# aswanthabam/JPEG_Decoder

Hardware: AMD Instinct MI355X
Metric: Mpixels/s decoded (IDCT+colour) (higher is better)
Workload: dtype f32; 1 GPU; stream of 4096x4096 baseline 4:4:4 images, 32 images per step (one launch) per GPU, coefficient blocks resident in HBM; sampling=4:4:4, parallelism=images sharded x1, no collective, launched_by=bench.py

## Files before the change

jpeg_decoder_amd/csrc/jb_huff.hip:

```cpp
#include <hip/hip_runtime.h>
#include <stdint.h>

#include "jb_huff_core.h"
#include "jb_kernels.h"

namespace {

constexpr uint32_t L = kJbhLanes;
constexpr int kMaxPasses = (int)L + 4;

__constant__ uint8_t kZz2Dev[64] = {0,   2,   16,  32,  18,  4,   6,   20,  34,  48, 64,  50,  36,  22,  8,   10,
                                    24,  38,  52,  66,  80,  96,  82,  68,  54,  40, 26,  12,  14,  28,  42,  56,
                                    70,  84,  98,  112, 114, 100, 86,  72,  58,  44, 30,  46,  60,  74,  88,  102,
                                    116, 118, 104, 90,  76,  62,  78,  92,  106, 120, 122, 108, 94,  110, 124, 126};

template <uint32_t kMaxChunk>
struct Lay {
  static constexpr uint32_t kRows = jbh_rows(kMaxChunk);
  static constexpr uint32_t kNcp = kMaxChunk * 8u / kJbCheckpointBits;
  static_assert(kNcp <= kJbCheckpoints, "records per chunk");
  static constexpr uint32_t off_stream = 0;
  static constexpr uint32_t off_cp = off_stream + kRows * L * 4u;
  static constexpr uint32_t off_xbit = off_cp + kNcp * L * 4u;
  static constexpr uint32_t off_xmeta = off_xbit + L * 4u;
  static constexpr uint32_t off_misc = off_xmeta + L * 4u;
  static constexpr uint32_t off_tab = off_misc + 256u;
  static uint32_t bytes(uint32_t n_tabs) { return off_tab + n_tabs * kJbT1Entries * 2u + kJbT2Tables * kJbT2Entries * 2u; }
};

struct ChunkGeo {
  uint32_t start, end;
  uint32_t seg;
  bool first, last;
};
__device__ __forceinline__ ChunkGeo chunk_geo(const JbHuffLaunch &p, const JbHuffImage &img, uint32_t gidx) {
  const JbChunkDesc cd = p.chunks[gidx];
  ChunkGeo x;
  x.seg = cd.seg & 0x7fffffffu;
  x.first = (cd.seg >> 31) != 0;
  uint32_t seg_end = p.starts[img.int_off + x.seg + 1];
  if (seg_end > img.scan_len) seg_end = img.scan_len;
  x.start = cd.start < seg_end ? cd.start : seg_end;
  x.end = x.start + img.chunk_bytes < seg_end ? x.start + img.chunk_bytes : seg_end;
  x.last = x.end == seg_end;
  return x;
}

template <uint32_t kRows>
__device__ __forceinline__ void load_stream(uint32_t *stream, const uint8_t *img_scan, uint32_t start, uint32_t tid) {
  const uint8_t *src = img_scan + (int32_t)jbh_base_byte(start);
#pragma unroll
  for (uint32_t q = 0; q < (kRows + 3u) / 4u; q++) {
    const uint4 v = *(const uint4 *)(src + 16u * q);
    const uint32_t d[4] = {v.x, v.y, v.z, v.w};
#pragma unroll
    for (uint32_t i = 0; i < 4; i++)
      if (4u * q + i < kRows) stream[(4u * q + i) * L + tid] = __builtin_bswap32(d[i]);
  }
}

__device__ __forceinline__ void load_tables(uint16_t *tab, const JbHuffLaunch &p, const JbHuffImage &img, uint32_t tid) {
  const JbHuffTables *set = p.tables + img.table_set;
  const uint4 *s1 = (const uint4 *)set->t1;
  uint4 *d = (uint4 *)tab;
  const uint32_t n1 = img.n_tabs * kJbT1Entries * 2u / 16u;
  for (uint32_t i = tid; i < n1; i += L) d[i] = s1[i];
  const uint4 *s2 = (const uint4 *)set->t2;
  constexpr uint32_t n2 = kJbT2Tables * kJbT2Entries * 2u / 16u;
  for (uint32_t i = tid; i < n2; i += L) d[n1 + i] = s2[i];
}

struct Seg {
  uint32_t f, n, d0, d1, d2;
};
__device__ __forceinline__ Seg seg_combine(const Seg &a, const Seg &b) {
  Seg r;
  r.f = a.f | b.f;
  r.n = b.f ? b.n : a.n + b.n;
  r.d0 = b.f ? b.d0 : a.d0 + b.d0;
  r.d1 = b.f ? b.d1 : a.d1 + b.d1;
  r.d2 = b.f ? b.d2 : a.d2 + b.d2;
  return r;
}
__device__ __forceinline__ Seg seg_shfl_up(const Seg &x, int off) {
  Seg r;
  r.f = __shfl_up(x.f, off);
  r.n = __shfl_up(x.n, off);
  r.d0 = __shfl_up(x.d0, off);
  r.d1 = __shfl_up(x.d1, off);
  r.d2 = __shfl_up(x.d2, off);
  return r;
}
__device__ __forceinline__ Seg seg_scan_wg(Seg x, uint32_t *scratch, uint32_t tid, Seg *total) {
  const uint32_t lane = tid & 63u, wave = tid >> 6;
#pragma unroll
  for (int off = 1; off < 64; off <<= 1) {
    const Seg t = seg_shfl_up(x, off);
    if (lane >= (uint32_t)off) x = seg_combine(t, x);
  }
  __syncthreads();
  if (lane == 63u) {
    uint32_t *s = scratch + wave * 5u;
    s[0] = x.f, s[1] = x.n, s[2] = x.d0, s[3] = x.d1, s[4] = x.d2;
  }
  __syncthreads();
  Seg run{0, 0, 0, 0, 0};
  Seg all{0, 0, 0, 0, 0};
#pragma unroll
  for (uint32_t w = 0; w < L / 64u; w++) {
    const uint32_t *s = scratch + w * 5u;
    const Seg t{s[0], s[1], s[2], s[3], s[4]};
    if (w < wave) run = seg_combine(run, t);
    all = seg_combine(all, t);
  }
  *total = all;
  return seg_combine(run, x);
}

__device__ __forceinline__ Seg fold_left_workgroups(const JbHuffLaunch &p, uint32_t w_first, uint32_t w_me, uint32_t *red, uint32_t tid) {
  if (tid < 8) red[tid] = 0;
  __syncthreads();
  uint32_t last_f = 0;
  for (uint32_t w = w_first + tid; w < w_me; w += L)
    if (p.wgsum[w].has_first) last_f = w - w_first + 1u;
  if (last_f) atomicMax(&red[0], last_f);
  __syncthreads();
  const uint32_t from = red[0];
  uint32_t a_n = 0, a0 = 0, a1 = 0, a2 = 0;
  for (uint32_t w = w_first + tid; w < w_me; w += L) {
    if (w - w_first + 1u >= from) {
      const JbWgSum s = p.wgsum[w];
      a_n += s.blocks, a0 += s.dc[0], a1 += s.dc[1], a2 += s.dc[2];
    }
  }
  if (a_n) atomicAdd(&red[1], a_n);
  if (a0) atomicAdd(&red[2], a0);
  if (a1) atomicAdd(&red[3], a1);
  if (a2) atomicAdd(&red[4], a2);
  __syncthreads();
  return Seg{from ? 1u : 0u, red[1], red[2], red[3], red[4]};
}
__device__ __forceinline__ Seg scan_left(const Seg &mine, const Seg &carry, uint32_t *scratch, uint32_t tid, Seg *total) {
  const Seg incl = seg_scan_wg(mine, scratch, tid, total);
  Seg left = seg_shfl_up(incl, 1);
  if ((tid & 63u) == 0) {
    left = Seg{0, 0, 0, 0, 0};
    for (uint32_t w = 0; w < (tid >> 6); w++) {
      const uint32_t *s = scratch + w * 5u;
      left = seg_combine(left, Seg{s[0], s[1], s[2], s[3], s[4]});
    }
  }
  return seg_combine(carry, left);
}

}

constexpr uint32_t kMet = 0x80000000u;

template <uint32_t kMaxChunk>
__global__ __launch_bounds__(kJbHuffLanes) void jb_huff_sync_kernel(const JbHuffLaunch p, const int launch) {
  using Ly = Lay<kMaxChunk>;
  extern __shared__ __attribute__((aligned(16))) uint8_t lds[];
  uint32_t *const stream = (uint32_t *)(lds + Ly::off_stream);
  uint32_t *const cpst = (uint32_t *)(lds + Ly::off_cp);
  uint32_t *const xbit = (uint32_t *)(lds + Ly::off_xbit);
  uint32_t *const xmeta = (uint32_t *)(lds + Ly::off_xmeta);
  uint32_t *const misc = (uint32_t *)(lds + Ly::off_misc);
  uint16_t *const tab = (uint16_t *)(lds + Ly::off_tab);
  const uint32_t tid = threadIdx.x;
  const JbHuffWg wg = p.sync_wgs[blockIdx.x];
  const JbHuffImage img = p.images[wg.image];
  const uint32_t ci = wg.first_chunk + tid - kJbWarmChunks;
  const bool owned = tid >= kJbWarmChunks && ci < img.n_chunks;
  const bool active = ci < img.n_chunks && (owned || launch == 0);
  const uint32_t gidx = img.state_off + (ci < img.n_chunks ? ci : img.n_chunks - 1u);
  const ChunkGeo g = chunk_geo(p, img, gidx);
  const uint32_t u0 = jbh_u_of_bit(g.start, g.start * 8u), u_end = u0 + (g.end - g.start) * 8u;
  const size_t n_all = p.n_chunks_total;

  JbChunkState entry{g.start * 8u, 0u}, exitst{0u, 0u};
  bool changed = active;
  if (launch > 0) {
    bool c0 = false;
    JbChunkState ne{0u, 0u};
    if (tid == kJbWarmChunks && owned && !g.first) {
      ne = p.exit[gidx - 1u];
      const JbChunkState en = p.entry[gidx];
      c0 = ne.bitpos != en.bitpos || ((ne.meta ^ en.meta) & 0xffffu) != 0;
    }
    if (!__syncthreads_or(c0)) return;
    entry = p.entry[gidx];
    exitst = p.exit[gidx];
    changed = c0;
    if (c0) entry = JbChunkState{ne.bitpos, ne.meta & 0xffffu};
  }
  load_tables(tab, p, img, tid);
  if (active) load_stream<Ly::kRows>(stream, p.scan + img.scan_off, g.start, tid);
#pragma unroll
  for (uint32_t i = 0; i < Ly::kNcp; i++) cpst[i * L + tid] = launch > 0 ? p.cps[i * n_all + gidx] : 0xffffffffu;
  __syncthreads();

  JbhCtx cx;
  cx.scol = stream + tid;
  cx.tab = tab;
  cx.zz2 = nullptr;
  cx.lut_ac = img.lut_ac, cx.lut_dc = img.lut_dc, cx.lut_comp = img.lut_comp;
  cx.nb4 = img.nb * 4u;
  cx.blk_bytes = img.blk_bytes;
  cx.t2_first = img.n_tabs * kJbT1Entries;
  uint32_t *const cpl = cpst + tid;

  for (int pass = 0; pass < kMaxPasses; pass++) {
    if (__builtin_amdgcn_ballot_w64(changed) != 0) {
      JbhLane st;
      {
        const uint32_t bit = entry.bitpos < g.start * 8u ? g.start * 8u : entry.bitpos;
        const uint32_t u = jbh_u_of_bit(g.start, bit);
        st.u = (changed && u < u_end) ? u : u_end;
        st.k = entry.meta & 0xffu;
        st.blk4 = ((entry.meta >> 8) & 0xffu) * 4u;
        if (st.k > 63u) st.k = 0;
        if (st.blk4 >= cx.nb4) st.blk4 = 0;
        st.nblk = 0;
      }
      uint32_t none = 0;
      while (st.u < u_end) {
        const uint32_t up = st.u;
        (void)jbh_step<false>(cx, st, none, none, none, nullptr, 0u);
        if (((st.u ^ up) >> 8) != 0) {
          uint32_t *rec = cpl + ((st.u >> 8) - 1u) * L;
          const uint32_t s = jbh_pack_state(st), old = *rec;
          const bool met = (st.u < u_end) & (((old ^ s) & 0xfffffu) == 0);
          *rec = met ? old : s;
          st.u = met ? (kMet | ((st.u >> 8) - 1u)) : st.u;
        }
      }
      JBH_TRACE_PASS_END(pass);
      if (changed) {
        if (st.u >= kMet) {
          const uint32_t met_i = st.u & 0xffu;
          const uint32_t dn = st.nblk - (cpl[met_i * L] >> 20);
          for (uint32_t i = met_i; i < Ly::kNcp; i++) cpl[i * L] += dn << 20;
          exitst.meta = (exitst.meta & 0xffffu) | ((((exitst.meta >> 16) + dn) & 0xffffu) << 16);
        } else {
          exitst.bitpos = jbh_bit_of_u(g.start, st.u);
          exitst.meta = st.k | (st.blk4 << 6) | ((st.nblk & 0xffffu) << 16);
        }
      }
    }
    xbit[tid] = exitst.bitpos;
    xmeta[tid] = exitst.meta & 0xffffu;
    __syncthreads();
    changed = false;
    if (active && !g.first && tid > (launch == 0 ? 0u : kJbWarmChunks)) {
      const uint32_t nbit = xbit[tid - 1u], nmeta = xmeta[tid - 1u];
      if (nbit != entry.bitpos || nmeta != (entry.meta & 0xffffu)) {
        entry = JbChunkState{nbit, nmeta};
        changed = true;
      }
    }
    if (!__syncthreads_or(changed)) break;
  }
  if (owned) {
    p.entry[gidx] = entry;
    p.exit[gidx] = exitst;
#pragma unroll
    for (uint32_t i = 0; i < Ly::kNcp; i++) p.cps[i * n_all + gidx] = cpl[i * L];
  }
  Seg mine{0, 0, 0, 0, 0};
  if (owned) {
    mine.f = g.first ? 1u : 0u;
    mine.n = (exitst.meta >> 16) + (g.first ? g.seg * img.ri * img.nb : 0u);
  }
  Seg total;
  (void)seg_scan_wg(mine, misc + 16, tid, &total);
  if (tid == 0) {
    JbWgSum *o = p.wgsum + img.wg0 + wg.first_chunk / kJbOwnChunks;
    o->has_first = total.f;
    o->blocks = total.n;
  }
}

template <uint32_t kMaxChunk>
__global__ __launch_bounds__(kJbHuffLanes) void jb_huff_write_kernel(const JbHuffLaunch p) {
  using Ly = Lay<kMaxChunk>;
  extern __shared__ __attribute__((aligned(16))) uint8_t lds[];
  uint32_t *const stream = (uint32_t *)(lds + Ly::off_stream);
  uint32_t *const misc = (uint32_t *)(lds + Ly::off_misc);
  uint16_t *const tab = (uint16_t *)(lds + Ly::off_tab);
  const uint32_t tid = threadIdx.x;
  const JbHuffWg wg = p.wgs[blockIdx.x];
  const JbHuffImage img = p.images[wg.image];
  const uint32_t ci = wg.first_chunk + tid;
  const bool active = tid < kJbOwnChunks && ci < img.n_chunks;
  const uint32_t gidx = img.state_off + (active ? ci : img.n_chunks - 1u);
  const ChunkGeo g = chunk_geo(p, img, gidx);
  const uint32_t u0 = jbh_u_of_bit(g.start, g.start * 8u), u_end = u0 + (g.end - g.start) * 8u;
  const uint32_t bpi = img.ri * img.nb;

  load_tables(tab, p, img, tid);
  if (tid < 16) ((uint32_t *)misc)[tid] = ((const uint32_t *)kZz2Dev)[tid];
  if (active) load_stream<Ly::kRows>(stream, p.scan + img.scan_off, g.start, tid);

  uint32_t err = 0;
  JbChunkState entry{g.start * 8u, 0u}, want{0u, 0u};
  uint32_t block = g.seg * bpi;
  if (img.needs_sync) {
    Seg mine{0, 0, 0, 0, 0};
    if (active) {
      want = p.exit[gidx];
      mine.f = g.first ? 1u : 0u;
      mine.n = (want.meta >> 16) + (g.first ? g.seg * bpi : 0u);
      if (!g.first) {
        const JbChunkState prev = p.exit[gidx - 1u];
        const JbChunkState en = p.entry[gidx];
        entry = JbChunkState{prev.bitpos, prev.meta & 0xffffu};
        if (en.bitpos != prev.bitpos || ((en.meta ^ prev.meta) & 0xffffu) != 0) err |= 4u;
      }
    }
    const Seg carry = fold_left_workgroups(p, img.wg0, img.wg0 + wg.first_chunk / kJbOwnChunks, misc + 40, tid);
    Seg total;
    const Seg left = scan_left(mine, carry, misc + 16, tid, &total);
    if (!g.first) block = left.n;
  }
  __syncthreads();

  JbhCtx cx;
  cx.scol = stream + tid;
  cx.tab = tab;
  cx.zz2 = (const uint8_t *)misc;
  cx.lut_ac = img.lut_ac, cx.lut_dc = img.lut_dc, cx.lut_comp = img.lut_comp;
  cx.nb4 = img.nb * 4u;
  cx.blk_bytes = img.blk_bytes;
  cx.t2_first = img.n_tabs * kJbT1Entries;

  uint32_t block_end = (g.seg + 1u) * img.ri < img.n_mcus ? (g.seg + 1u) * bpi : img.n_mcus * img.nb;
  if (block_end > img.n_blocks) block_end = img.n_blocks;
  JbhLane st;
  const bool overran = active && entry.bitpos > g.end * 8u;
  {
    const uint32_t bit = entry.bitpos < g.start * 8u ? g.start * 8u : entry.bitpos;
    const uint32_t u = jbh_u_of_bit(g.start, bit);
    st.u = u < u_end ? u : u_end;
    st.k = entry.meta & 0xffu;
    st.blk4 = ((entry.meta >> 8) & 0xffu) * 4u;
    if (st.k > 63u) st.k = 0;
    if (st.blk4 >= cx.nb4) st.blk4 = 0;
    st.nblk = 0;
  }
  const uint32_t k_in = st.k;
  uint32_t dc0 = 0, dc1 = 0, dc2 = 0;
  uint8_t *const coef = (uint8_t *)p.coef + img.coef_off;
  bool live = active && st.u < u_end && block < block_end;
  while (live) {
    if (jbh_step<true>(cx, st, dc0, dc1, dc2, coef, block)) {
      err |= 1u;
      live = false;
    } else {
      live = st.u < u_end && block + st.nblk < block_end;
    }
  }
  JBH_TRACE_PASS_END(0);
  if (active) {
    if (g.last) {
      if (block + st.nblk != block_end || st.k != 0 || st.u > u_end || overran) err |= 2u;
    } else if (img.needs_sync) {
      if (jbh_bit_of_u(g.start, st.u) != want.bitpos || (st.k | (st.blk4 << 6) | ((st.nblk & 0xffffu) << 16)) != want.meta) err |= 4u;
    }
    if (err) atomicOr(p.status + wg.image, err);
    JbChunkDc o;
    o.dc[0] = dc0, o.dc[1] = dc1, o.dc[2] = dc2;
    o.first_block = block + (k_in != 0 ? 1u : 0u);
    o.count = err ? 0u : st.nblk + (st.k != 0 ? 1u : 0u) - (k_in != 0 ? 1u : 0u);
    o.pad[0] = o.pad[1] = o.pad[2] = 0;
    p.chunk_dc[gidx] = o;
  }
  if (img.needs_sync) {
    Seg mine{0, 0, 0, 0, 0};
    if (active) mine = Seg{g.first ? 1u : 0u, 0u, dc0, dc1, dc2};
    Seg total;
    (void)seg_scan_wg(mine, misc + 16, tid, &total);
    if (tid == 0) {
      JbWgSum *o = p.wgsum + img.wg0 + wg.first_chunk / kJbOwnChunks;
      o->dc[0] = total.d0, o->dc[1] = total.d1, o->dc[2] = total.d2;
    }
  }
}

__global__ __launch_bounds__(kJbHuffLanes) void jb_huff_dc_kernel(const JbHuffLaunch p) {
  extern __shared__ __attribute__((aligned(16))) uint8_t lds[];
  uint32_t *const misc = (uint32_t *)lds;
  const uint32_t tid = threadIdx.x;
  const JbHuffWg wg = p.wgs[blockIdx.x];
  const JbHuffImage img = p.images[wg.image];
  const uint32_t ci = wg.first_chunk + tid;
  const bool active = tid < kJbOwnChunks && ci < img.n_chunks;
  const uint32_t gidx = img.state_off + (active ? ci : img.n_chunks - 1u);
  const bool first = (p.chunks[gidx].seg >> 31) != 0;
  JbChunkDc cd = p.chunk_dc[gidx];
  if (!active) cd.count = 0;
  uint32_t p0 = 0, p1 = 0, p2 = 0;
  if (img.needs_sync) {
    Seg mine{0, 0, 0, 0, 0};
    if (active) mine = Seg{first ? 1u : 0u, 0u, cd.dc[0], cd.dc[1], cd.dc[2]};
    const Seg carry = fold_left_workgroups(p, img.wg0, img.wg0 + wg.first_chunk / kJbOwnChunks, misc + 40, tid);
    Seg total;
    const Seg left = scan_left(mine, carry, misc + 16, tid, &total);
    if (!first) p0 = left.d0, p1 = left.d1, p2 = left.d2;
  }
  uint8_t *const coef = (uint8_t *)p.coef + img.coef_off;
  uint32_t pos4 = (cd.first_block % img.nb) * 4u;
  uint32_t bad = 0;
  constexpr uint32_t kBatch = 24;
  for (uint32_t i = 0; i < cd.count; i += kBatch) {
    int32_t diff[kBatch];
#pragma unroll
    for (uint32_t q = 0; q < kBatch; q++) diff[q] = i + q < cd.count ? *(const int16_t *)(coef + (size_t)jbh_mul24(cd.first_block + i + q, img.blk_bytes)) : 0;
#pragma unroll
    for (uint32_t q = 0; q < kBatch; q++) {
      if (i + q < cd.count) {
        const uint32_t c = jbh_ubfe(img.lut_comp, pos4, 4);
        const uint32_t pr = (c == 0 ? p0 : c == 1 ? p1 : p2) + (uint32_t)diff[q];
        bad |= (pr + 32768u) > 65535u ? 1u : 0u;
        p0 = c == 0 ? pr : p0;
        p1 = c == 1 ? pr : p1;
        p2 = c == 2 ? pr : p2;
        *(int16_t *)(coef + (size_t)jbh_mul24(cd.first_block + i + q, img.blk_bytes)) = (int16_t)pr;
        pos4 = pos4 + 4u == img.nb * 4u ? 0u : pos4 + 4u;
      }
    }
  }
  if (bad) atomicOr(p.status + wg.image, 1u);
}

__global__ __launch_bounds__(256) void jb_huff_fetch_kernel(uint4 *dst, const uint4 *src, uint32_t n16) {
  for (uint32_t i = blockIdx.x * 256u + threadIdx.x; i < n16; i += gridDim.x * 256u) dst[i] = src[i];
}
__global__ __launch_bounds__(256) void jb_huff_zero_kernel(uint4 *dst, uint64_t n16, uint4 *small, uint32_t small16) {
  const uint4 z = make_uint4(0, 0, 0, 0);
  if (blockIdx.x == 0 && threadIdx.x < small16) small[threadIdx.x] = z;
  for (uint64_t i = (uint64_t)blockIdx.x * 256u + threadIdx.x; i < n16; i += (uint64_t)gridDim.x * 256u) dst[i] = z;
}
hipError_t jbk_huff_zero(void *d_dst, size_t bytes, hipStream_t stream, void *d_small, size_t small_bytes) {
  (void)hipGetLastError();
  const uint64_t n16 = (bytes + 15) / 16;
  uint64_t blocks = (n16 + 255u) / 256u;
  if (blocks > 8192u) blocks = 8192u;
  const uint32_t small16 = d_small ? (uint32_t)((small_bytes + 15) / 16) : 0u;
  if (small16 > 256u) return hipErrorInvalidValue;
  hipLaunchKernelGGL(jb_huff_zero_kernel, dim3((unsigned)(blocks ? blocks : 1u)), dim3(256), 0, stream, (uint4 *)d_dst, n16, (uint4 *)d_small, small16);
  return hipGetLastError();
}
hipError_t jbk_huff_fetch(void *d_dst, const void *h_pinned_src, size_t bytes, hipStream_t stream) {
  (void)hipGetLastError();
  const uint32_t n16 = (uint32_t)((bytes + 15) / 16);
  unsigned blocks = (n16 + 255u) / 256u;
  if (blocks > 1024u) blocks = 1024u;
  hipLaunchKernelGGL(jb_huff_fetch_kernel, dim3(blocks ? blocks : 1u), dim3(256), 0, stream, (uint4 *)d_dst, (const uint4 *)h_pinned_src, n16);
  return hipGetLastError();
}

hipError_t jbk_huff_launch(const JbHuffLaunch &p, hipStream_t stream) {
  (void)hipGetLastError();
  const dim3 block(kJbHuffLanes);
  const uint32_t n_tabs = p.max_tabs < 2u ? 2u : p.max_tabs > kJbMaxTabs ? kJbMaxTabs : p.max_tabs;
  const bool small = p.max_chunk_bytes <= 64u;
  const unsigned lds = small ? Lay<64>::bytes(n_tabs) : Lay<128>::bytes(n_tabs);
  if (p.n_sync_wgs > 0) {
    const int launches = p.sync_launches > 0 ? p.sync_launches : kJbSyncLaunches;
    for (int l = 0; l < launches; l++) {
      if (small) hipLaunchKernelGGL(jb_huff_sync_kernel<64>, dim3((unsigned)p.n_sync_wgs), block, lds, stream, p, l);
      else hipLaunchKernelGGL(jb_huff_sync_kernel<128>, dim3((unsigned)p.n_sync_wgs), block, lds, stream, p, l);
    }
  }
  if (p.n_wgs > 0) {
    if (small) hipLaunchKernelGGL(jb_huff_write_kernel<64>, dim3((unsigned)p.n_wgs), block, lds, stream, p);
    else hipLaunchKernelGGL(jb_huff_write_kernel<128>, dim3((unsigned)p.n_wgs), block, lds, stream, p);
    hipLaunchKernelGGL(jb_huff_dc_kernel, dim3((unsigned)p.n_wgs), block, 256, stream, p);
  }
  return hipGetLastError();
}
```

jpeg_decoder_amd/csrc/jb_huff_core.h:

```cpp
#pragma once
#include <stdint.h>

#include "jb_huff.h"

#if defined(__HIPCC__)
#define JBH_FN __host__ __device__ inline __attribute__((always_inline))
#else
#define JBH_FN inline
#endif

JBH_FN uint32_t jbh_alignbit(uint32_t hi, uint32_t lo, uint32_t sh) {
#if defined(__HIP_DEVICE_COMPILE__)
  return __builtin_amdgcn_alignbit(hi, lo, sh);
#else
  return (uint32_t)(((((uint64_t)hi) << 32) | lo) >> (sh & 31u));
#endif
}
JBH_FN uint32_t jbh_ubfe(uint32_t v, uint32_t off, uint32_t width) {
#if defined(__HIP_DEVICE_COMPILE__)
  return __builtin_amdgcn_ubfe(v, off, width);
#else
  off &= 31u, width &= 31u;
  return width ? (v >> off) & ((1u << width) - 1u) : 0u;
#endif
}
JBH_FN int32_t jbh_sbfe(uint32_t v, uint32_t off, uint32_t width) {
#if defined(__HIP_DEVICE_COMPILE__)
  return __builtin_amdgcn_sbfe((int32_t)v, off, width);
#else
  off &= 31u, width &= 31u;
  if (!width) return 0;
  const uint32_t f = (v >> off) & ((1u << width) - 1u);
  return (int32_t)(f << (32u - width)) >> (32u - width);
#endif
}

JBH_FN uint32_t jbh_mul24(uint32_t a, uint32_t b) { return (a & 0xffffffu) * (b & 0xffffffu); }

#ifndef JBH_TRACE_STEP
#define JBH_TRACE_STEP() ((void)0)
#define JBH_TRACE_PASS_END(pass) ((void)0)
#endif

constexpr uint32_t kJbhLanes = (uint32_t)kJbHuffLanes;
constexpr uint32_t jbh_rows(uint32_t chunk_bytes) { return chunk_bytes / 4u + 3u; }

JBH_FN uint32_t jbh_base_byte(uint32_t start) { return (start & ~3u) - 4u; }
JBH_FN uint32_t jbh_u_of_bit(uint32_t start, uint32_t bit) { return bit - 8u * jbh_base_byte(start) - 1u; }
JBH_FN uint32_t jbh_bit_of_u(uint32_t start, uint32_t u) { return u + 8u * jbh_base_byte(start) + 1u; }

struct JbhCtx {
  const uint32_t *scol;
  const uint16_t *tab;
  const uint8_t *zz2;
  uint32_t lut_ac, lut_dc, lut_comp;
  uint32_t nb4;
  uint32_t blk_bytes;
  uint32_t t2_first;
};
struct JbhLane {
  uint32_t u;
  uint32_t k;
  uint32_t blk4;
  uint32_t nblk;
};

template <bool kStore>
JBH_FN bool jbh_step(const JbhCtx &cx, JbhLane &st, uint32_t &dc0, uint32_t &dc1, uint32_t &dc2, uint8_t *coef, uint32_t block0) {
  JBH_TRACE_STEP();
  const uint32_t u = st.u;
  const uint32_t j = jbh_ubfe(u, 5, 27);
  const uint32_t w = jbh_alignbit(cx.scol[j * kJbhLanes], cx.scol[j * kJbhLanes + kJbhLanes], ~u);
  const bool isdc = st.k == 0;
  const uint32_t tix = jbh_ubfe(isdc ? cx.lut_dc : cx.lut_ac, st.blk4, 4);
  uint32_t e = cx.tab[(tix << kJbT1Bits) + (w >> (32 - kJbT1Bits))];
  if (e - 1u < 31u)
    e = cx.tab[cx.t2_first + ((e - 1u) << kJbT2Bits) + ((w >> 16) & (kJbT2Entries - 1u))];
  const uint32_t total = e & 31u, size = (e >> 5) & 15u, adv = e >> 9;
  const uint32_t k1 = st.k + adv;
  const bool bad = e == 0 || (k1 - 65u) < 17u;
  if (kStore) {
    const int32_t x = jbh_sbfe(w, 32u - total, size);
    const int32_t val = x - (int32_t)(((1u << size) - 1u) ^ (uint32_t)(x >> 31));
    const uint32_t c = jbh_ubfe(cx.lut_comp, st.blk4, 4);
    const uint32_t dcv = (isdc && !bad) ? (uint32_t)val : 0u;
    dc0 += c == 0 ? dcv : 0u;
    dc1 += c == 1 ? dcv : 0u;
    dc2 += c == 2 ? dcv : 0u;
    if (!bad && (isdc || size != 0))
      *(int16_t *)(coef + (jbh_mul24(block0 + st.nblk, cx.blk_bytes) + cx.zz2[k1 - 1u])) = (int16_t)val;
  }
  const uint32_t k2 = k1 - ((size == 0 && !isdc) ? 1u : 0u);
  const bool done = k2 >= 64u;
  const bool next = done || bad;
  st.k = next ? 0u : k2;
  st.nblk += (done && !bad) ? 1u : 0u;
  const uint32_t b4 = st.blk4 + (next ? 4u : 0u);
  st.blk4 = b4 == cx.nb4 ? 0u : b4;
  st.u = u + (bad ? 1u : total);
  return bad;
}

JBH_FN uint32_t jbh_pack_state(const JbhLane &st) { return st.u | (st.k << 11) | (st.blk4 << 15) | (st.nblk << 20); }

#include <string.h>

inline uint16_t jbh_entry_(bool is_ac, int len, int sym) {
  if (!is_ac) {
    if (sym > 11) return 0;
    return (uint16_t)((len + sym) | (sym << 5) | (1 << 9));
  }
  const int run = sym >> 4, size = sym & 15;
  if (size > 10) return 0;
  if (sym == 0) return (uint16_t)(len | (kJbAdvEob << 9));
  if (sym == 0xf0) return (uint16_t)(len | (17 << 9));
  return (uint16_t)((len + size) | (size << 5) | ((run + 1) << 9));
}

inline bool jb_huff_fill_table_impl_(const uint8_t counts[17], const uint8_t *symbols, bool is_ac, JbHuffTables *set, uint32_t tix, uint32_t n_tabs,
                                     uint32_t *n_t2) {
  uint16_t *t1 = set->t1[tix];
  memset(t1, 0, sizeof set->t1[0]);
  uint32_t code = 0;
  int k = 0;
  int32_t sub_of_prefix = -1;
  uint32_t sub_prefix = 0;
  for (int len = 1; len <= 16; len++) {
    for (int i = 0; i < counts[len]; i++, k++, code++) {
      if (code >= (1u << len)) return false;
      const uint16_t e = jbh_entry_(is_ac, len, symbols[k]);
      if (len <= kJbT1Bits) {
        const uint32_t first = code << (kJbT1Bits - len);
        for (uint32_t q = 0; q < (1u << (kJbT1Bits - len)); q++) t1[first + q] = e;
      } else {
        const uint32_t prefix = code >> (len - kJbT1Bits);
        if (sub_of_prefix < 0 || sub_prefix != prefix) {
          if (*n_t2 >= kJbT2Tables) return false;
          sub_of_prefix = (int32_t)(*n_t2)++;
          sub_prefix = prefix;
          memset(set->t2[sub_of_prefix], 0, sizeof set->t2[0]);
          t1[prefix] = (uint16_t)(sub_of_prefix + 1);
        }
        const uint32_t rest = len - kJbT1Bits;
        const uint32_t first = (code & ((1u << rest) - 1u)) << (kJbT2Bits - rest);
        for (uint32_t q = 0; q < (1u << (kJbT2Bits - rest)); q++) set->t2[sub_of_prefix][first + q] = e;
      }
    }
    code <<= 1;
  }
  return true;
}
```

Before: 644,700 Mpixels/s.

## Compact live chunks into dense wave work lists for Huffman resync passes

Each resync pass now packs the chunks that still need re-decoding into an LDS work list through a ballot and prefix count, so the unresolved chunks are handled by densely packed lanes instead of scattered ones. Whole waves with no work skip the decode loop, and a per-block, per-pass rotation spreads the work across waves. Decoder state is handed back through LDS (pack/unpack into 32 bits), and the exit-state fix-up runs after a barrier. This adds two extra barriers per pass and LDS traffic, and it reuses the xbit/xmeta scratch space, which relies on the 11-bit u field holding.

```diff
diff --git a/jpeg_decoder_amd/csrc/jb_huff.hip b/jpeg_decoder_amd/csrc/jb_huff.hip
--- a/jpeg_decoder_amd/csrc/jb_huff.hip
+++ b/jpeg_decoder_amd/csrc/jb_huff.hip
@@ -155,7 +155,22 @@
 
 }
 
-constexpr uint32_t kMet = 0x80000000u;
+__device__ __forceinline__ uint32_t pack_list(bool live, uint32_t c, uint8_t *list, uint32_t *cnt, uint32_t tid) {
+  const uint64_t m = __builtin_amdgcn_ballot_w64(live);
+  const uint32_t lane = tid & 63u, wave = tid >> 6;
+  if (lane == 0) cnt[wave] = (uint32_t)__builtin_popcountll(m);
+  __syncthreads();
+  uint32_t base = 0, n = 0;
+#pragma unroll
+  for (uint32_t w = 0; w < L / 64u; w++) {
+    const uint32_t k = cnt[w];
+    base += w < wave ? k : 0u;
+    n += k;
+  }
+  if (live) list[base + (uint32_t)__builtin_popcountll(m & ((1ull << lane) - 1ull))] = (uint8_t)c;
+  __syncthreads();
+  return n;
+}
 
 template <uint32_t kMaxChunk>
 __global__ __launch_bounds__(kJbHuffLanes) void jb_huff_sync_kernel(const JbHuffLaunch p, const int launch) {
@@ -201,7 +216,7 @@
   __syncthreads();
 
   JbhCtx cx;
-  cx.scol = stream + tid;
+  cx.scol = stream;
   cx.tab = tab;
   cx.zz2 = nullptr;
   cx.lut_ac = img.lut_ac, cx.lut_dc = img.lut_dc, cx.lut_comp = img.lut_comp;
@@ -209,43 +224,65 @@
   cx.blk_bytes = img.blk_bytes;
   cx.t2_first = img.n_tabs * kJbT1Entries;
   uint32_t *const cpl = cpst + tid;
+  uint32_t *const rstate = xbit;
+  uint16_t *const rend = (uint16_t *)xmeta;
+  uint8_t *const rlist = (uint8_t *)xmeta + 2u * L;
+  uint32_t *const rcnt = (uint32_t *)((uint8_t *)xmeta + 3u * L);
 
   for (int pass = 0; pass < kMaxPasses; pass++) {
-    if (__builtin_amdgcn_ballot_w64(changed) != 0) {
+    bool live = false;
+    if (changed) {
       JbhLane st;
-      {
-        const uint32_t bit = entry.bitpos < g.start * 8u ? g.start * 8u : entry.bitpos;
-        const uint32_t u = jbh_u_of_bit(g.start, bit);
-        st.u = (changed && u < u_end) ? u : u_end;
-        st.k = entry.meta & 0xffu;
-        st.blk4 = ((entry.meta >> 8) & 0xffu) * 4u;
-        if (st.k > 63u) st.k = 0;
-        if (st.blk4 >= cx.nb4) st.blk4 = 0;
-        st.nblk = 0;
-      }
-      uint32_t none = 0;
-      while (st.u < u_end) {
-        const uint32_t up = st.u;
-        (void)jbh_step<false>(cx, st, none, none, none, nullptr, 0u);
-        if (((st.u ^ up) >> 8) != 0) {
-          uint32_t *rec = cpl + ((st.u >> 8) - 1u) * L;
-          const uint32_t s = jbh_pack_state(st), old = *rec;
-          const bool met = (st.u < u_end) & (((old ^ s) & 0xfffffu) == 0);
-          *rec = met ? old : s;
-          st.u = met ? (kMet | ((st.u >> 8) - 1u)) : st.u;
+      const uint32_t bit = entry.bitpos < g.start * 8u ? g.start * 8u : entry.bitpos;
+      const uint32_t u = jbh_u_of_bit(g.start, bit);
+      st.u = u < u_end ? u : u_end;
+      st.k = entry.meta & 0xffu;
+      st.blk4 = ((entry.meta >> 8) & 0xffu) * 4u;
+      if (st.k > 63u) st.k = 0;
+      if (st.blk4 >= cx.nb4) st.blk4 = 0;
+      st.nblk = 0;
+      rstate[tid] = jbh_pack_state(st);
+      rend[tid] = (uint16_t)u_end;
+      live = st.u < u_end;
+    }
+    const uint32_t n = pack_list(live, tid, rlist, rcnt, tid);
+    const uint32_t rot = ((blockIdx.x * 0x9e3779b1u) ^ ((uint32_t)pass * 0x85ebca6bu)) >> 30;
+    const uint32_t wi = (tid + 64u * (4u - rot)) & (L - 1u);
+    if (wi - (wi & 63u) < n) {
+      if (wi < n) {
+        const uint32_t c = rlist[wi];
+        JbhLane st = jbh_unpack_state(rstate[c]);
+        const uint32_t ue = rend[c];
+        uint32_t lim = ue;
+        cx.scol = stream + c;
+        uint32_t *const cpc = cpst + c;
+        uint32_t none = 0;
+        while (st.u < lim) {
+          const uint32_t up = st.u;
+          (void)jbh_step<false>(cx, st, none, none, none, nullptr, 0u);
+          if (((st.u ^ up) >> 8) != 0) {
+            uint32_t *rec = cpc + ((st.u >> 8) - 1u) * L;
+            const uint32_t s = jbh_pack_state(st), old = *rec;
+            const bool met = (st.u < ue) & (((old ^ s) & 0xfffffu) == 0);
+            *rec = met ? old : s;
+            lim = met ? 0u : lim;
+          }
         }
+        rstate[c] = jbh_pack_state(st);
       }
       JBH_TRACE_PASS_END(pass);
-      if (changed) {
-        if (st.u >= kMet) {
-          const uint32_t met_i = st.u & 0xffu;
-          const uint32_t dn = st.nblk - (cpl[met_i * L] >> 20);
-          for (uint32_t i = met_i; i < Ly::kNcp; i++) cpl[i * L] += dn << 20;
-          exitst.meta = (exitst.meta & 0xffffu) | ((((exitst.meta >> 16) + dn) & 0xffffu) << 16);
-        } else {
-          exitst.bitpos = jbh_bit_of_u(g.start, st.u);
-          exitst.meta = st.k | (st.blk4 << 6) | ((st.nblk & 0xffffu) << 16);
-        }
+    }
+    __syncthreads();
+    if (changed) {
+      const JbhLane st = jbh_unpack_state(rstate[tid]);
+      if (st.u < u_end) {
+        const uint32_t met_i = (st.u >> 8) - 1u;
+        const uint32_t dn = st.nblk - (cpl[met_i * L] >> 20);
+        for (uint32_t i = met_i; i < Ly::kNcp; i++) cpl[i * L] += dn << 20;
+        exitst.meta = (exitst.meta & 0xffffu) | ((((exitst.meta >> 16) + dn) & 0xffffu) << 16);
+      } else {
+        exitst.bitpos = jbh_bit_of_u(g.start, st.u);
+        exitst.meta = st.k | (st.blk4 << 6) | ((st.nblk & 0xffffu) << 16);
       }
     }
     xbit[tid] = exitst.bitpos;
diff --git a/jpeg_decoder_amd/csrc/jb_huff_core.h b/jpeg_decoder_amd/csrc/jb_huff_core.h
--- a/jpeg_decoder_amd/csrc/jb_huff_core.h
+++ b/jpeg_decoder_amd/csrc/jb_huff_core.h
@@ -102,6 +102,15 @@
 }
 
 JBH_FN uint32_t jbh_pack_state(const JbhLane &st) { return st.u | (st.k << 11) | (st.blk4 << 15) | (st.nblk << 20); }
+static_assert(56u + 8u * kJbChunkBytes + 27u < 2048u, "u fits 11 bits");
+JBH_FN JbhLane jbh_unpack_state(uint32_t s) {
+  JbhLane st;
+  st.u = s & 0x7ffu;
+  st.k = (s >> 11) & 63u;
+  st.blk4 = (s >> 15) & 0x1cu;
+  st.nblk = s >> 20;
+  return st;
+}
 
 #include <string.h>
 
```

After: 645,200 Mpixels/s, median of 3. No clear change (+0.1%).
